# debbiemarkslab/EVcouplings

Hardware: AMD Instinct MI355X
Metric: plmc L-BFGS iterations/sec (PLM fit, synthetic MSA) (higher is better)
Workload: dtype f32 (forward: f16 hi/lo split couplings on the 2:4 sparse MFMA, f32 accumulation -- in the last iterations of a fit 39-bit fixed-point couplings as five int8 digit planes, exact; backward: 24-bit fixed-point residuals as three int8 digit planes on the int8 MFMA (32-bit / four there), exact int32 acc; 1 GPU; headline: synthetic MSA L=300 q=21 N=50000, theta=0.8, lambda_h=0.01, lambda_J=59.8; parallelism=single GPU

## Files before the change

evcouplings_amd/csrc/plm_host.cpp:

```cpp
#include "../../include/plm_hip.h"
#include "plm_internal.h"

#include <algorithm>
#include <chrono>
#include <cmath>
#include <cstdarg>
#include <cstdio>
#include <cstdlib>
#include <cstring>
#include <string>
#include <vector>

namespace {

thread_local std::string g_err;

int fail(int code, const char *fmt, ...) {
    char buf[512];
    va_list ap;
    va_start(ap, fmt);
    vsnprintf(buf, sizeof buf, fmt, ap);
    va_end(ap);
    g_err = buf;
    return code;
// ... 18 lines not shown
        hipError_t e__ = (expr);                                                                   \
        if (e__ != hipSuccess)                                                                     \
            return fail(e__ == hipErrorOutOfMemory ? PLM_ENOMEM : PLM_EDEVICE, "%s failed: %s (%s:%d)", \
                        #expr, hipGetErrorString(e__), __FILE__, __LINE__);                        \
    } while (0)
#define PLM_TRY(expr)                  \
    do {                               \
        int rc__ = (expr);             \
        if (rc__ != PLM_OK) return rc__; \
    } while (0)

double now_s() {
    return std::chrono::duration<double>(std::chrono::steady_clock::now().time_since_epoch()).count();
}

int check_device(int device) {
    int n = 0;
    if (hipGetDeviceCount(&n) != hipSuccess || n <= 0)
        return fail(PLM_EDEVICE, "no HIP device visible (libplm_hip has no CPU path)");
    if (device < 0 || device >= n) return fail(PLM_EINVAL, "device %d out of range (%d visible)", device, n);
    hipDeviceProp_t prop;
    HIP_TRY(hipGetDeviceProperties(&prop, device));
    if (strncmp(prop.gcnArchName, "gfx950", 6) != 0)
        return fail(PLM_EDEVICE, "device %d is %s; this library is built for gfx950 only", device, prop.gcnArchName);
    HIP_TRY(hipSetDevice(device));
    return PLM_OK;
}

}
int plm_check_device(int device) { return check_device(device); }
namespace {

int cluster_threshold(double theta_id, int L, int conv) {
    if (conv & PLM_CONV_THRESHOLD_F32) {
        const float t = (float)(1.0 - theta_id);
        const float need = (1.0f - t) * (float)L;
        return (int)std::ceil(need);
    }
    return (int)std::ceil(theta_id * (double)L - 1e-9);
}

}
PlmOptions plm_options_from_env() {
    PlmOptions o;
    if (const char *e = getenv("PLM_BWD_PLANES")) o.bwd_planes = atoi(e) == 4 ? 4 : 3;
    if (const char *e = getenv("PLM_KSPLIT")) o.ksplit = std::max(1, atoi(e));
    if (const char *e = getenv("PLM_JEXP_BIAS")) o.jexp_bias = atoi(e);
    if (const char *e = getenv("PLM_BWD_KERNEL")) o.bwd_kernel = atoi(e) ? 1 : 0;
    if (const char *e = getenv("PLM_FWD_KERNEL")) o.fwd_kernel = atoi(e) ? 1 : 0;
    if (const char *e = getenv("PLM_FWD_ACCURATE")) o.fwd_mode = atoi(e) ? 1 : 0;
    if (const char *e = getenv("PLM_VP_FLOOR")) o.vp_floor = atof(e);
    if (const char *e = getenv("PLM_VP_REL")) o.vp_rel = atof(e);
    if (const char *e = getenv("PLM_VP_HESS_POS")) o.vp_hess_pos = atoi(e);
    if (const char *e = getenv("PLM_ACC_FACTOR")) o.acc_factor = atof(e);
    o.debug = getenv("PLM_DEBUG") != nullptr;
    o.debug_vp = getenv("PLM_DEBUG_VP") != nullptr;
    return o;
}
namespace {

int pick_ksplit(const PlmDims &d, const PlmOptions &opt, int nplanes, int *out) {
    const int ks_min = std::max(1, (d.nst128 + 1022) / 1023);
    const int ks_max = std::max(ks_min, std::max(1, std::min(16, d.nst128 / 8)));
    if ((int64_t)((d.nst128 + ks_min - 1) / ks_min) * PLM_BWD_KSTEP * 128 * 128 >= ((int64_t)1 << 31))
        return fail(PLM_EUNSUPPORTED, "%d sequences: no admissible K split of the backward GEMM", d.N);
    const double beta = (2.0 * nplanes * (double)d.nmf * d.nnfl * 1024.0 / 12e12) / ((double)d.nst128 * 1.3e-6);
    int best = ks_min;
    double best_cost = 1e300;
    for (int ks = ks_min; ks <= ks_max; ks++) {
        const int groups_per_xcd = (d.ncol_tiles * nplanes * ks + 7) / 8;
        const double cost = (double)((groups_per_xcd * d.nrow_tiles + 31) / 32) / ks + beta * ks;
        if (cost < best_cost * 0.98) { best_cost = cost; best = ks; }
    }
    if (opt.ksplit) best = std::max(ks_min, std::min(ks_max, opt.ksplit));
    *out = best;
    return PLM_OK;
}

int make_dims(const plm_problem_t &p, const PlmOptions &opt, PlmDims *out) {
    PlmDims d;
    memset(&d, 0, sizeof d);
    if (p.n_seqs <= 0 || p.n_sites <= 1) return fail(PLM_EINVAL, "need n_seqs > 0 and n_sites > 1");
    if (!plm_q_supported(p.n_states))
        return fail(PLM_EUNSUPPORTED, "alphabet size %d outside 2..32", p.n_states);
    const int nshards = p.n_shards > 0 ? p.n_shards : 1;
    if (p.shard < 0 || p.shard >= nshards) return fail(PLM_EINVAL, "shard %d outside 0..%d", p.shard, nshards - 1);
    d.N = p.n_seqs;
    d.L = p.n_sites;
    d.Qc = p.n_states;
    d.Q = plm_q_template(p.n_states);
    d.Np = (d.N + PLM_SEQ_TILE - 1) / PLM_SEQ_TILE * PLM_SEQ_TILE;
    d.nb16 = (d.L + 15) / 16;
    d.Lp16 = d.nb16 * 16;
    d.nu = (d.L + 31) / 32;
    d.Lp32 = d.nu * 32;
    d.nksteps = d.nu * PLM_FWD_TILES(d.Q);
    d.nssteps = d.Np / 32;
    d.nst128 = d.Np / PLM_BWD_KSTEP;
    d.nplanes = (p.epsilon > 0 && p.epsilon < 1e-4) ? 4 : 3;
    if (opt.bwd_planes) d.nplanes = opt.bwd_planes;
    d.jexp_bias = opt.jexp_bias;
    const float qmax = d.nplanes == 4 ? PLM_R_QMAX4 : PLM_R_QMAX3;
    d.rscale = qmax;
    d.gscale = 1.0f / (qmax * (float)PLM_BWD_ONEHOT_VALUE);
    d.nstiles = d.Np / PLM_SEQ_TILE;
    plm_pick_tile(d.Q, &d.FM, &d.FN);
// ... 275 lines not shown
                                 plm_reg_parts(d), c->scal, c->st));
    c->n_evals++;
    return PLM_OK;
}

bool vp_enabled(const plm_ctx *c) {
    return !(c->prob.flags & PLM_FLAG_JOINT_LBFGS) && (c->d.nshards == 1 || c->d.sharded) && c->prob.lambda_h > 0;
}
int vp_alloc(plm_ctx *c) {
    if (c->hj) return PLM_OK;
    const size_t nsites = (size_t)std::max(std::max(1, (c->d.b16_hi - c->d.b16_lo) * 16),
                                           std::min(c->d.L, c->d.own_hi * 16) - c->d.h_site0);
    PLM_TRY(dalloc((char **)&c->hj, plm_hj_bytes(c->d)));
    PLM_TRY(dalloc((char **)&c->hpart, plm_hpart_bytes(c->d)));
    PLM_TRY(dalloc((char **)&c->gpart, plm_gpart_bytes(c->d)));
    PLM_TRY(dalloc((char **)&c->dpart, plm_gpart_bytes(c->d)));
    PLM_TRY(dalloc(&c->hg2, nsites));
    PLM_TRY(dalloc(&c->hinv, nsites * c->d.Q * c->d.Q));
    PLM_TRY(dalloc(&c->h64, 2 * plm_h64_stride(c->d)));
    PLM_TRY(dalloc(&c->hcnt, plm_h64_stride(c->d)));
    c->hcnt_valid = false;
    PLM_TRY(dalloc((char **)&c->vp_flag, sizeof(PlmVpState)));
    HIP_TRY(hipMemsetAsync(c->vp_flag, 0, sizeof(PlmVpState), c->st));
    for (auto &e : c->vp_ev) HIP_TRY(hipEventCreate(&e));
    for (auto &e : c->gemm_ev) HIP_TRY(hipEventCreate(&e));
    c->vp_hess_age = -1;
    return PLM_OK;
}
int vp_counts(plm_ctx *c) {
    if (!c->hcnt_valid) {
        HIP_TRY(plm_launch_site_counts(c->d, c->msa_cm, c->w, c->hcnt, c->st));
        c->hcnt_valid = true;
    }
    return PLM_OK;
}
int vp_stage1(plm_ctx *c) {
    const PlmDims &d = c->d;
    PLM_TRY(vp_counts(c));
    if (d.sharded) {
        PLM_TRY(ctx_collective(c, PLM_COLL_ALLTOALL, x_rectangles(c), c->xhalo, c->x_send.data(), c->x_recv.data()));
        HIP_TRY(plm_launch_maxabs2(c->x + d.nh_pad_l, d.n_local - d.nh_pad_l, c->xhalo,
                                   d.nx_halo * (int64_t)PLM_BLOCK_FLOATS(d), c->maxbits, c->jexp, d.jexp_bias, c->st));
        HIP_TRY(plm_launch_expand(d, c->x, c->xhalo, c->jexp, c->Bt, c->fwd_accurate ? 1 : 0, c->st));
    } else {
        HIP_TRY(plm_launch_maxabs(d, c->x, c->maxbits, c->jexp, c->st));
        HIP_TRY(plm_launch_expand(d, c->x, nullptr, c->jexp, c->Bt, c->fwd_accurate ? 1 : 0, c->st));
    }
    if (c->gemm_ev[0]) HIP_TRY(hipEventRecord(c->gemm_ev[0], c->st));
    HIP_TRY(plm_launch_forward_store(d, c->msa_rm, c->Bt, c->jexp, c->hj, c->fwd_accurate, c->st));
    HIP_TRY(plm_launch_h64_init(d, c->x, c->h64, c->st));
    return PLM_OK;
}
int vp_counts(plm_ctx *c);
int vp_step_and_residuals(plm_ctx *c, bool refresh) {
    const PlmDims &d = c->d;
    PLM_TRY(vp_counts(c));
    const int full = (refresh || c->vp_hess_age < 0) ? 1 : 0;
    HIP_TRY(plm_launch_hpass(d, c->hj, c->msa_rm, c->w, c->h64, 0, full ? 2 : 1, c->fwd_accurate, nullptr, nullptr, c->hpart,
                             c->gpart, c->dpart, nullptr, PLM_VP_ALWAYS, c->st));
    HIP_TRY(plm_launch_hsolve(d, c->hpart, c->gpart, full, c->x, c->h64, c->prob.lambda_h, 1, c->hinv, c->hg2, c->scal + 5, 0.0,
                              0.0, nullptr, 0, c->hcnt, c->dpart, c->st));
    if (full) c->vp_hess_age = 0;
    HIP_TRY(plm_launch_hpass(d, c->hj, c->msa_rm, c->w, c->h64, 1, 1, c->fwd_accurate, c->Rt, c->fx_part, c->hpart, c->gpart,
                             nullptr, nullptr, PLM_VP_ALWAYS, c->st));
    HIP_TRY(plm_launch_hsolve(d, c->hpart, c->gpart, 0, c->x, c->h64, c->prob.lambda_h, 0, c->hinv, c->hg2, c->scal + 5, 0.0,
                              0.0, nullptr, 0, c->hcnt, c->dpart, c->st));
    return PLM_OK;
}
int vp_chain(plm_ctx *c, int npos, int hess_upto, int expected_last, double tol2) {
    const PlmDims &d = c->d;
    for (int k = 0; k < npos; k++) {
        const int pos = c->vp_pos++;
        const bool hess = pos < hess_upto || pos > expected_last || c->vp_hess_age < 0;
        HIP_TRY(plm_launch_hpass(d, c->hj, c->msa_rm, c->w, c->h64, 0, hess ? 2 : 1, c->fwd_accurate, nullptr, nullptr, c->hpart,
                                 c->gpart, c->dpart, c->vp_flag, PLM_VP_PASS, c->st));
        HIP_TRY(plm_launch_hpass(d, c->hj, c->msa_rm, c->w, c->h64, 1, 1, c->fwd_accurate, c->Rt, c->fx_part, c->hpart, c->gpart,
                                 nullptr, c->vp_flag, PLM_VP_PASS_RT, c->st));
        HIP_TRY(plm_launch_hsolve(d, c->hpart, c->gpart, hess ? 2 : 0, c->x, c->h64, c->prob.lambda_h, 1, c->hinv, c->hg2,
                                  c->scal + 5, tol2, c->vp_floor2, c->vp_flag, 1, c->hcnt, c->dpart, c->st));
        if (hess && pos < 32) c->vp_hess_mask |= 1u << pos;
        if (hess && c->vp_hess_age < 0) c->vp_hess_age = 0;
    }
    return PLM_OK;
}
int vp_stage3(plm_ctx *c, bool conditional, float *gout = nullptr, int mode = 2) {
    const PlmDims &d = c->d;
    if (!gout) gout = c->g;
    if (c->gemm_ev[1]) HIP_TRY(hipEventRecord(c->gemm_ev[1], c->st));
    if (d.nblk_own > 0 || !d.sharded)
        HIP_TRY(plm_launch_backward(d, c->msa_cm, c->Rt, c->G, (conditional && !d.sharded) ? c->vp_flag : nullptr, c->st));
    if (c->gemm_ev[2]) HIP_TRY(hipEventRecord(c->gemm_ev[2], c->st));
    if (d.sharded) {
        HIP_TRY(plm_launch_pack_g(d, c->G, c->gsend, c->st));
        PLM_TRY(ctx_collective(c, PLM_COLL_ALLTOALL, c->gsend, c->ghalo, c->g_send.data(), c->g_recv.data()));
    }
    PLM_TRY(group_norms(c));
    HIP_TRY(plm_launch_assemble(d, c->G, d.ksplit, d.sharded ? c->ghalo : nullptr, c->x, gout, c->prob.lambda_h,
                                c->prob.lambda_j, c->reg_part, mode, 0.f, c->pair_n2, (float)c->prob.lambda_group, c->st));
    if (mode == 2)
        HIP_TRY(plm_launch_finish_fx(d, c->fx_part, c->n_fx_part(), nullptr, 0, c->reg_part, plm_reg_parts(d), c->scal,
                                     c->st));
    return PLM_OK;
}
int ctx_eval_vp_enqueue(plm_ctx *c, double tol2) {
    const PlmDims &d = c->d;
    PLM_TRY(vp_stage1(c));
    if (c->vp_ev_pending) c->vp_ev_pending = false;
    HIP_TRY(hipEventRecord(c->vp_ev[0], c->st));
    const int c_prev = c->vp_c_prev;
    if (c->vp_hess_age >= 0) c->vp_hess_age++;
    const bool stale = c->vp_hess_age < 0 || c->vp_hess_age >= 32;
    HIP_TRY(plm_launch_vp_reset(c->vp_flag, (c_prev == 0 && !stale) ? 1 : 0, c->scal + 5, c->st));
    c->vp_pos = 0;
    c->vp_extra = 0;
    c->vp_hess_mask = 0;
    c->vp_last_gh2 = INFINITY;
    int hess_upto = c_prev >= 2 ? c_prev : (stale ? 1 : 0);
    if (c->opt.vp_hess_pos >= 0) hess_upto = std::min(hess_upto, std::max(c->opt.vp_hess_pos, c->vp_hess_age < 0 ? 1 : 0));
    PLM_TRY(vp_chain(c, std::min(14, c_prev + 3), hess_upto, c_prev, tol2));
    HIP_TRY(plm_launch_fields_to_x(d, c->h64, c->vp_flag, c->x, c->st));
    HIP_TRY(plm_launch_hpass(d, c->hj, c->msa_rm, c->w, c->h64, 1, 0, c->fwd_accurate, c->Rt, c->fx_part, nullptr, nullptr, nullptr,
                             c->vp_flag, PLM_VP_FINAL, c->st));
    HIP_TRY(hipEventRecord(c->vp_ev[1], c->st));
    c->vp_ev_pending = true;
    PLM_TRY(vp_stage3(c, true));
    c->n_evals++;
    return PLM_OK;
// ... 1025 lines not shown
            snprintf(res->status_msg, sizeof res->status_msg, "%s", status_text(status));
    }
    return PLM_OK;
}

int plm_ctx_scores(plm_ctx_t *c, float *fn_host, float *cn_host) {
    if (!c || !fn_host || !cn_host) return fail(PLM_EINVAL, "NULL argument");
    HIP_TRY(hipSetDevice(c->device));
    const PlmDims &d = c->d;
    float *fn_dev = c->canon + d.n_canon;
    PLM_TRY(canon_full(c, c->x));
    PlmDims dc = d;
    dc.Q = d.Qc;
    if (d.gap_mode) {
        HIP_TRY(plm_launch_fn(dc, c->canon + (size_t)d.L * d.Qc, fn_dev, 1, 1, c->st));
    } else {
        HIP_TRY(plm_launch_fn(dc, c->canon + (size_t)d.L * d.Qc, fn_dev, (d.conv & PLM_CONV_FN_NO_GAP) ? 1 : 0, 0, c->st));
    }
    HIP_TRY(hipMemcpyAsync(fn_host, fn_dev, sizeof(float) * d.L * d.L, hipMemcpyDeviceToHost, c->st));
    HIP_TRY(hipStreamSynchronize(c->st));
    const int L = d.L;
    std::vector<double> col(L, 0.0);
    double tot = 0;
    for (int i = 0; i < L; i++)
        for (int j = 0; j < L; j++) {
            col[j] += fn_host[(size_t)i * L + j];
            tot += fn_host[(size_t)i * L + j];
        }
    const double mean = tot / ((double)L * (L - 1));
    for (int j = 0; j < L; j++) col[j] /= (double)(L - 1);
    for (int i = 0; i < L; i++)
        for (int j = 0; j < L; j++)
            cn_host[(size_t)i * L + j] =
                (i == j) ? 0.f : (float)((double)fn_host[(size_t)i * L + j] - col[i] * col[j] / mean);
    return PLM_OK;
}

int plm_ctx_time_field_positions(plm_ctx_t *c, int32_t reps, float *out_ms) {
    if (!c || !out_ms || reps <= 0) return fail(PLM_EINVAL, "bad argument");
    if (!c->have_weights) return fail(PLM_EINVAL, "weights not set");
    if (!vp_enabled(c) || !c->hj) return fail(PLM_EINVAL, "no stored potentials: plm_ctx_time_kernels on a variable-projection context first");
    HIP_TRY(hipSetDevice(c->device));
    const PlmDims &d = c->d;
    c->eval_valid = false;
    ctx_set_accurate(c, false);
    PLM_TRY(vp_counts(c));
    hipEvent_t ev[3] = {nullptr, nullptr, nullptr};
    for (auto &e : ev) HIP_TRY(hipEventCreate(&e));
    double acc[2] = {0, 0};
    int rc = PLM_OK;
    for (int r = 0; r < reps && rc == PLM_OK; r++) {
        float ms;
        hipError_t e = hipEventRecord(ev[0], c->st);
        if (e == hipSuccess) e = plm_launch_hpass(d, c->hj, c->msa_rm, c->w, c->h64, 0, 2, 0, nullptr, nullptr, c->hpart, c->gpart, c->dpart,
                                                  nullptr, PLM_VP_ALWAYS, c->st);
        if (e == hipSuccess) e = plm_launch_hsolve(d, c->hpart, c->gpart, 1, c->x, c->h64, c->prob.lambda_h, 1, c->hinv, c->hg2, c->scal + 5,
                                                   0.0, 0.0, nullptr, 0, c->hcnt, c->dpart, c->st);
        if (e == hipSuccess) e = hipEventRecord(ev[1], c->st);
        if (e == hipSuccess) e = plm_launch_hpass(d, c->hj, c->msa_rm, c->w, c->h64, 1, 1, 0, c->Rt, c->fx_part, c->hpart, c->gpart, nullptr,
                                                  nullptr, PLM_VP_ALWAYS, c->st);
        if (e == hipSuccess) e = plm_launch_hsolve(d, c->hpart, c->gpart, 0, c->x, c->h64, c->prob.lambda_h, 0, c->hinv, c->hg2, c->scal + 5,
                                                   0.0, 0.0, nullptr, 0, c->hcnt, c->dpart, c->st);
        if (e == hipSuccess) e = hipEventRecord(ev[2], c->st);
        if (e == hipSuccess) e = hipEventSynchronize(ev[2]);
        if (e == hipSuccess && hipEventElapsedTime(&ms, ev[0], ev[1]) == hipSuccess) acc[0] += ms;
        if (e == hipSuccess && hipEventElapsedTime(&ms, ev[1], ev[2]) == hipSuccess) acc[1] += ms;
        if (e != hipSuccess) rc = fail(PLM_EDEVICE, "field position timing: %s", hipGetErrorString(e));
    }
    for (auto &e : ev) (void)hipEventDestroy(e);
    c->vp_hess_age = 0;
    out_ms[0] = (float)(acc[0] / reps);
    out_ms[1] = (float)(acc[1] / reps);
    return rc;
}

int plm_ctx_time_kernels(plm_ctx_t *c, int32_t reps, float *out_ms) {
    if (!c || !out_ms || reps <= 0) return fail(PLM_EINVAL, "bad argument");
    if (!c->have_weights) return fail(PLM_EINVAL, "weights not set");
    if (c->d.nshards > 1 && !c->d.sharded) return fail(PLM_EUNSUPPORTED, "kernel timing runs on 1-shard or sharded-state contexts");
    HIP_TRY(hipSetDevice(c->device));
    c->eval_valid = false;
    ctx_set_accurate(c, false);
    const PlmDims &d = c->d;
    struct Events {
        hipEvent_t e[6] = {nullptr, nullptr, nullptr, nullptr, nullptr, nullptr};
        ~Events() { for (auto &x : e) if (x) (void)hipEventDestroy(x); }
    } evs;
    hipEvent_t (&ev)[6] = evs.e;
    for (auto &e : ev) HIP_TRY(hipEventCreate(&e));
    double acc[PLM_K_COUNT] = {0};
    const bool vp = vp_enabled(c);
    if (vp) PLM_TRY(vp_alloc(c));
    for (int r = 0; r < reps; r++) {
        float ms;
        HIP_TRY(hipEventRecord(ev[0], c->st));
        if (d.sharded) {
            HIP_TRY(plm_launch_maxabs2(c->x + d.nh_pad_l, d.n_local - d.nh_pad_l, c->xhalo,
                                       d.nx_halo * (int64_t)PLM_BLOCK_FLOATS(d), c->maxbits, c->jexp, d.jexp_bias, c->st));
            HIP_TRY(plm_launch_expand(d, c->x, c->xhalo, c->jexp, c->Bt, c->fwd_accurate ? 1 : 0, c->st));
        } else {
            HIP_TRY(plm_launch_maxabs(d, c->x, c->maxbits, c->jexp, c->st));
            HIP_TRY(plm_launch_expand(d, c->x, nullptr, c->jexp, c->Bt, c->fwd_accurate ? 1 : 0, c->st));
        }
        HIP_TRY(hipEventRecord(ev[1], c->st));
        if (vp) {
            HIP_TRY(plm_launch_forward_store(d, c->msa_rm, c->Bt, c->jexp, c->hj, 0, c->st));
            HIP_TRY(hipEventRecord(ev[2], c->st));
// ... 465 lines not shown
```

evcouplings_amd/csrc/plm_internal.h:

```cpp
#pragma once
#include <stdint.h>
#include <stddef.h>
#include <hip/hip_runtime.h>

#define PLM_MAX_SHARDS 16
#define PLM_PAD_STATE 127
#define PLM_SEQ_TILE 256
#define PLM_R_EXP 14
#define PLM_BWD_MAXPLANES 4
#define PLM_R_QMAX3 8355000.0f
#define PLM_R_QMAX4 2138000000.0f
#define PLM_BWD_KSTEP 128
#define PLM_BWDW_COLS 9
#define PLM_BWD_ONEHOT_VALUE (-128)

#define PLM_FWD_NG(Q) (((Q) + 2) / 4)
#define PLM_FWD_SPU(Q) (4 * PLM_FWD_NG(Q))
#define PLM_FWD_TILES(Q) (5 * PLM_FWD_NG(Q))

struct PlmDims {
    int N, L, Q;
    int Qc;
    int Np;
    int nb16;
    int Lp16;
    int nu;
    int Lp32;
    int nksteps;
    int nssteps;
    int nst128;
    int nplanes;
    float rscale;
    float gscale;
    int nstiles;
    int FM, FN;
    int nmf;
    int nshards, shard;
    int blk_per_shard;
    int shard_base, shard_rem;
    int b16_lo, b16_hi;
    int nnfl;
    int ksplit;
    int nrow_tiles, ncol_tiles;
    int fwd_w;
    int bwd_w;
    int64_t nbp;
    int64_t nh_pad;
    int64_t n_native;
    int64_t n_canon;
    int gap_mode;
    int jexp_bias;
    int conv;
    double theta;
    int sharded;
    int own_lo, own_hi;
    int nblk_own;
    int h_site0;
    int64_t bp_base;
    int64_t np_own;
    int64_t nh_pad_l;
    int64_t n_local;
    int64_t nx_halo;
    int64_t ng_halo;
    int ntri;
    int own_base[PLM_MAX_SHARDS], oth_base[PLM_MAX_SHARDS];
};

struct PlmOptions {
    int bwd_planes = 0;
    int ksplit = 0;
    int fwd_kernel = -1;
    int bwd_kernel = -1;
    int jexp_bias = 0;
    int fwd_mode = -1;
    double acc_factor = 8.0;
    double vp_rel = 1e-4;
    int vp_hess_pos = -1;
    double vp_floor = 2e-7;
    bool debug = false;
    bool debug_vp = false;
};
PlmOptions plm_options_from_env();

static inline __host__ __device__ int plm_shard_lo(const PlmDims &d, int r) {
    const int small = d.nshards - d.shard_rem;
    return r * d.shard_base + (r > small ? r - small : 0);
}
static inline __host__ __device__ int plm_shard_cnt(const PlmDims &d, int r) {
    return d.shard_base + (r >= d.nshards - d.shard_rem ? 1 : 0);
}
static inline __host__ __device__ int plm_shard_of(const PlmDims &d, int b) {
    const int small = d.nshards - d.shard_rem, nsmall = small * d.shard_base;
    if (b < nsmall) return d.shard_base > 0 ? b / d.shard_base : 0;
    return small + (b - nsmall) / (d.shard_base + 1);
}
static inline __host__ __device__ int64_t plm_bp_index(int I, int J, int nb16) {
    return (int64_t)I * nb16 - (int64_t)I * (I - 1) / 2 + (J - I);
}
static inline __host__ __device__ int plm_pair_owner(const PlmDims &d, int I, int sI, int sJ) {
    return ((I - plm_shard_lo(d, sI)) & 1) ? sJ : sI;
}
static inline __host__ __device__ int64_t plm_half_blocks(const PlmDims &d, int p) {
    return d.shard < p ? (int64_t)((d.nblk_own + 1) / 2) * plm_shard_cnt(d, p) : (int64_t)(plm_shard_cnt(d, p) / 2) * d.nblk_own;
}
static inline __host__ __device__ int64_t plm_pair_local(const PlmDims &d, int I, int J, int *halo) {
    if (halo) *halo = -1;
    if (!d.sharded) return plm_bp_index(I, J, d.nb16);
    const int sI = plm_shard_of(d, I), sJ = plm_shard_of(d, J);
    if (sI == d.shard && sJ == d.shard) {
        const int r = I - d.own_lo;
        return (int64_t)r * d.nblk_own - (int64_t)r * (r - 1) / 2 + (J - I);
    }
    if (sI != d.shard && sJ != d.shard) return -1;
    const int p = sI == d.shard ? sJ : sI;
    const int idx = ((I - plm_shard_lo(d, sI)) >> 1) * plm_shard_cnt(d, sJ) + (J - plm_shard_lo(d, sJ));
    if (plm_pair_owner(d, I, sI, sJ) == d.shard) return (int64_t)d.ntri + d.own_base[p] + idx;
    if (halo) *halo = d.oth_base[p] + idx;
    return -1;
}
static inline __host__ __device__ void plm_half_pair(const PlmDims &d, int p, bool mine, int64_t k, int *I, int *J) {
    const int np = plm_shard_cnt(d, p);
    if (d.shard < p) {
        *I = d.own_lo + 2 * (int)(k / np) + (mine ? 0 : 1);
        *J = plm_shard_lo(d, p) + (int)(k % np);
    } else {
        *I = plm_shard_lo(d, p) + 2 * (int)(k / d.nblk_own) + (mine ? 1 : 0);
        *J = d.own_lo + (int)(k % d.nblk_own);
    }
}
static inline __host__ __device__ void plm_pair_of_local(const PlmDims &d, int64_t k, int *I, int *J) {
// ... 139 lines not shown
```

evcouplings_amd/csrc/plm_kernels.hip:

```cpp
#include "../../include/plm_hip.h"
#include "plm_internal.h"
#include <math.h>
#include <stdlib.h>
#include <string.h>
#include <mutex>
#include <utility>

typedef _Float16 half8 __attribute__((ext_vector_type(8)));
typedef _Float16 half4 __attribute__((ext_vector_type(4)));
typedef _Float16 half16 __attribute__((ext_vector_type(16)));
typedef float f32x4 __attribute__((ext_vector_type(4)));
typedef int i32x4 __attribute__((ext_vector_type(4)));
typedef unsigned int u32;

#ifndef PLM_DMA_STAGGER_FWD
#define PLM_DMA_STAGGER_FWD 4
#endif
#ifndef PLM_DMA_STAGGER_BWD
#define PLM_DMA_STAGGER_BWD 0
#endif
typedef unsigned long long u64;
#ifndef PLM_ASYNC_A
#define PLM_ASYNC_A 1
#endif
// ... 1124 lines not shown
__host__ __device__ constexpr int plm_qc_min(int Q) { return Q == 4 ? 2 : Q == 5 ? 5 : Q == 20 ? 6 : Q == 21 ? 21 : 22; }
#ifndef PLM_HESS_SAMPLE
#define PLM_HESS_SAMPLE 32
#endif
#ifndef PLM_NEWTON_CAP
#define PLM_NEWTON_CAP 3.0
#endif
__device__ __forceinline__ float sum_over_g(float v) {
    unsigned u = __float_as_uint(v);
    auto a = __builtin_amdgcn_permlane32_swap(u, u, false, false);
    v = __uint_as_float(a[0]) + __uint_as_float(a[1]);
    u = __float_as_uint(v);
    auto b = __builtin_amdgcn_permlane16_swap(u, u, false, false);
    return __uint_as_float(b[0]) + __uint_as_float(b[1]);
}
__device__ __forceinline__ float log_unbiased(float z) {
    const float l2 = __builtin_amdgcn_logf(z);
    return __builtin_fmaf(l2, -1.904654323148236e-9f, l2 * 0.693147182464599609375f);
}
__device__ __forceinline__ float sel_eq(int x, int a, float if_ne, float if_eq) {
    float out;
    asm("v_cmp_eq_u32 vcc, %1, %2\n\tv_cndmask_b32 %0, %3, %4, vcc" : "=v"(out) : "s"(a), "v"(x), "v"(if_ne), "v"(if_eq) : "vcc");
    return out;
}
__device__ __forceinline__ void sel_eq2(int x, int a, float ne0, float eq0, float ne1, float eq1, float &o0, float &o1) {
    asm("v_cmp_eq_u32 vcc, %2, %3\n\tv_cndmask_b32 %0, %4, %5, vcc\n\tv_cndmask_b32 %1, %6, %7, vcc"
        : "=&v"(o0), "=&v"(o1) : "s"(a), "v"(x), "v"(ne0), "v"(eq0), "v"(ne1), "v"(eq1) : "vcc");
}
__global__ void k_sum_partials(const double *__restrict__ p, int n, double *out);
struct HpassArgs {
    const float4 *hj;
    const int8_t *msa_rm;
    const float *w;
    const double *h;
    int hstride;
    char *Rt;
    double *fx_part;
    float *hpart;
    double *gpart;
    float rscale;
    double *dpart;
    const int *state;
    int cond;
    int sel;
};
__device__ __forceinline__ bool vp_runs(const int *state, int cond) {
    if (!state || cond == PLM_VP_ALWAYS) return true;
    const PlmVpState *S = (const PlmVpState *)state;
    if (cond == PLM_VP_FINAL) return S->final_skip == 0;
    if (S->done) return false;
    return cond == PLM_VP_PASS_RT ? S->want_rt != 0 : S->want_rt == 0;
}
#define PLM_HESS_PARTS(Q) (((Q) == 20 || (Q) == 21) ? 3 : 1)
template <int Q> __host__ __device__ constexpr int hess_entry0(int a) { return a * Q - a * (a - 1) / 2; }
template <int Q> __host__ __device__ constexpr int hess_row_begin(int part) {
    if (part <= 0) return 0;
    if (part >= PLM_HESS_PARTS(Q)) return Q;
    int a = 0;
    while (a < Q && hess_entry0<Q>(a) * PLM_HESS_PARTS(Q) < part * (Q * (Q + 1) / 2)) a++;
    return a;
}
template <int Q> __host__ __device__ constexpr int hess_part_entries() {
    int m = 0;
    for (int p = 0; p < PLM_HESS_PARTS(Q); p++) {
        const int n = hess_entry0<Q>(hess_row_begin<Q>(p + 1)) - hess_entry0<Q>(hess_row_begin<Q>(p));
        m = n > m ? n : m;
    }
    return m;
}
template <int Q, bool WRITE_RT, int STATS, bool XACT>
__global__ __launch_bounds__(512) void k_hpass(PlmDims d, HpassArgs A) {
    extern __shared__ __attribute__((aligned(16))) char smem[];
    constexpr int NH = (STATS == 2) ? Q * (Q + 1) / 2 : 0;
    constexpr int NSP = (STATS == 2) ? PLM_HESS_PARTS(Q) : 1;
    constexpr int NHP = (STATS == 2) ? hess_part_entries<Q>() : 0;
    if (!vp_runs(A.state, A.cond)) return;
    if (A.state) A.h += (size_t)((const PlmVpState *)A.state)->cur * A.hstride;
    const int tid = threadIdx.x, lane = tid & 63;
    const int wave = __builtin_amdgcn_readfirstlane(tid >> 6);
    const int ns1 = (d.nstiles + PLM_HESS_SAMPLE - 1) / PLM_HESS_SAMPLE;
    const int sel = A.sel;
    const int part = (int)blockIdx.x % NSP, bid = (int)blockIdx.x / NSP;
    int row_lo = 0, row_hi = Q;
    if constexpr (NSP > 1) {
        row_lo = part == 0 ? 0 : (part == 1 ? hess_row_begin<Q>(1) : hess_row_begin<Q>(2));
        row_hi = part == 0 ? hess_row_begin<Q>(1) : (part == 1 ? hess_row_begin<Q>(2) : Q);
    }
    const int ent_lo = row_lo * Q - row_lo * (row_lo - 1) / 2, ent_hi = row_hi * Q - row_hi * (row_hi - 1) / 2;
    const int nst = sel == 0 ? d.nstiles : (sel == 1 ? ns1 : d.nstiles - ns1);
    const int kt = bid % nst, b16l = bid / nst;
    if (A.state && A.cond == PLM_VP_PASS && b16l < PLM_VP_MAXBLK && ((const PlmVpState *)A.state)->quiet[b16l]) return;
    const int stile = sel == 0 ? kt : (sel == 1 ? kt * PLM_HESS_SAMPLE : kt + kt / (PLM_HESS_SAMPLE - 1) + 1);
    constexpr int HW = Q > 21 ? 2 : 8;
    constexpr bool sampled = STATS == 2, DIAG = STATS == 3 || (STATS == 2 && Q > 21);
    const int blk = b16l * d.nstiles + stile;
    const int b16 = d.b16_lo + b16l;
    const int r = lane & 15, g = lane >> 4;
    const int s_wave = stile * PLM_SEQ_TILE + wave * 32;
    const int gap = d.gap_mode;
    const int i = b16 * 16 + r;
    const bool site_ok = i < d.L;
    float hv[XACT ? 1 : Q], hl[XACT ? 1 : Q];
    double hd[XACT ? Q : 1];
    auto load_fields = [&](bool opaque) {
        u32 hoff = (u32)(site_ok ? i - d.h_site0 : 0) * Q;
        if (opaque) asm volatile("" : "+v"(hoff));
#pragma unroll
        for (int a = 0; a < Q; a++) {
            const double h64 = site_ok ? A.h[hoff + a] : 0.0;
            if constexpr (XACT) {
                hd[a] = h64;
            } else {
                hv[a] = (float)h64;
                hl[a] = (float)(h64 - (double)hv[a]);
            }
        }
    };
    constexpr bool LDSF = !WRITE_RT && !XACT && (STATS != 2 || Q > 21);
    constexpr size_t STAT_BYTES = (size_t)16 * (8 * Q * sizeof(double) * (DIAG ? 2 : 1) + HW * NHP * sizeof(float));
    float2 *lf = (float2 *)(smem + STAT_BYTES);
    constexpr bool FAST = !WRITE_RT && !XACT && (STATS == 1 || STATS == 3);
    if constexpr (LDSF) {
        for (int k = tid; k < 16 * Q; k += 512) {
            const int ii = b16 * 16 + k / Q;
            const double h64 = ii < d.L ? A.h[(size_t)(ii - d.h_site0) * Q + k % Q] : 0.0;
            const float hi = (float)h64;
            lf[k] = make_float2(hi, (float)(h64 - (double)hi));
        }
        __syncthreads();
    } else if constexpr (!WRITE_RT) load_fields(false);
    float fxl = 0.f;
    double *lg = (double *)smem + ((size_t)wave * 16 + r) * Q;
    double *ld = lg + (size_t)8 * 16 * Q;
    float *lh0 = (float *)((double *)smem + (size_t)8 * 16 * Q * (DIAG ? 2 : 1));
    float *ls = lh0 + ((size_t)wave * 16 + r) * NHP;
    if (STATS) {
        for (int k = lane; k < 16 * Q; k += 64) ((double *)smem)[(size_t)wave * 16 * Q + k] = 0.0;
        if constexpr (sampled)
            if (wave < HW)
                for (int k = lane; k < 16 * NHP; k += 64) lh0[(size_t)wave * 16 * NHP + k] = 0.f;
        if constexpr (DIAG)
            for (int k = lane; k < 16 * Q; k += 64) ((double *)smem)[(size_t)(8 + wave) * 16 * Q + k] = 0.0;
    }
    const char *hj_u = (const char *)(A.hj + ((size_t)blk * 8 + wave) * 2 * Q * 64);
    const u32 lane16 = (u32)lane * 16;
    int m_end = 2;
    asm volatile("" : "+s"(m_end));
#pragma nounroll
    for (int m = 0; m < m_end; m++) {
        if constexpr (WRITE_RT) load_fields(true);
        f32x4 acc[Q];
#pragma unroll
        for (int a = 0; a < Q; a++) {
            const float4 v = *(const float4 *)(hj_u + (size_t)(m * Q + a) * 1024 + lane16);
            acc[a] = (f32x4){v.x, v.y, v.z, v.w};
        }
        float wk[4];
        float izk[4];
        int xk[4];
#pragma unroll
        for (int reg = 0; reg < 4; reg++) {
            const int s = s_wave + 16 * m + 4 * g + reg;
            const int xi = A.msa_rm[(size_t)s * d.Lp32 + i];
            const bool skip = gap && xi == 0;
            const float ws = (skip || !site_ok) ? 0.f : A.w[s];
            float mx = -INFINITY, Z = 0.f, hx = 0.f, zo = 0.f;
            if constexpr (!XACT) {
                u32 foff = (u32)r * Q;
                if constexpr (LDSF) asm volatile("" : "+v"(foff));
#pragma unroll
                for (int a = 0; a < Q; a++) {
                    float fh, fl;
                    if constexpr (LDSF) {
                        const float2 f = lf[foff + a];
                        fh = f.x;
                        fl = f.y;
                    } else {
                        fh = hv[a];
                        fl = hl[a];
                    }
                    const float H = ((gap && a == 0) || (a >= plm_qc_min(Q) && a >= d.Qc)) ? -INFINITY : (acc[a][reg] + fl) + fh;
                    acc[a][reg] = H;
                    mx = fmaxf(mx, H);
                }
                if constexpr (FAST) {
                    const float mxl = -mx * 1.44269502f;
#pragma unroll
                    for (int a = 0; a < Q; a++) {
                        const float ev = __builtin_amdgcn_exp2f(__builtin_fmaf(acc[a][reg], 1.44269502f, mxl));
                        const float evo = sel_eq(xi, a, ev, 0.f);
                        acc[a][reg] = evo;
                        Z += ev;
                        zo += evo;
                    }
                } else {
#pragma unroll
                    for (int a = 0; a < Q; a++) {
                        const float H = acc[a][reg] - mx;
                        const float ev = __expf(H);
                        float evo;
                        sel_eq2(xi, a, hx, H, ev, 0.f, hx, evo);
                        acc[a][reg] = ev;
                        Z += ev;
                        zo += evo;
                    }
                }
            } else {
// ... 88 lines not shown
#endif
#ifndef PLM_EXP_NOLDS
                        if (g == 0) __builtin_amdgcn_ds_faddf(LDS_FPTR(&ls[idx]), v, 0, 0, false);
#else
                        fxl += v;
#endif
                        ++idx;
                    }
                }
#endif
            }
        }
        if constexpr (WRITE_RT) {
            __builtin_amdgcn_sched_barrier(0);
            const int s64 = stile * 4 + (wave >> 1);
            const int Gq = 2 * (wave & 1) + m;
            char *rt_u = A.Rt + rt_slot(d, 0, s64, b16l * Q, 0);
            const size_t rt_plane = (size_t)d.nst128 * d.nnfl * 2048;
            const u32 slot16 = (u32)(Gq * 16 + r) * 16;
#pragma unroll
            for (int reg = 0; reg < 4; reg++) {
                wk[reg] *= A.rscale;
                asm volatile("" : "+v"(xk[reg]));
            }
            const bool four = d.nplanes == 4;
            auto planes_of_state = [&](int a, u32 (&pl)[PLM_BWD_MAXPLANES]) {
                u32 x[4];
#pragma unroll
                for (int reg = 0; reg < 4; reg++)
                    x[reg] = digits_of(wk[reg] * acc[a][reg], four);
                planes_of4(x[0], x[1], x[2], x[3], pl);
            };
#pragma unroll
            for (int q4 = 0; q4 + 4 <= Q; q4 += 4) {
                u32 pl[4][PLM_BWD_MAXPLANES];
#pragma unroll
                for (int k = 0; k < 4; k++) planes_of_state(q4 + k, pl[k]);
                const u32 off = (u32)(q4 + g) * 2048 + slot16;
#pragma unroll
                for (int p = 0; p < PLM_BWD_MAXPLANES; p++) {
                    if (p >= d.nplanes) break;
                    auto s02 = __builtin_amdgcn_permlane32_swap(pl[0][p], pl[2][p], false, false);
                    auto s13 = __builtin_amdgcn_permlane32_swap(pl[1][p], pl[3][p], false, false);
                    auto t0 = __builtin_amdgcn_permlane16_swap(s02[0], s13[0], false, false);
                    auto t1 = __builtin_amdgcn_permlane16_swap(s02[1], s13[1], false, false);
                    *(uint4 *)(rt_u + p * rt_plane + off) = make_uint4(t0[0], t0[1], t1[0], t1[1]);
                }
                __builtin_amdgcn_sched_barrier(0);
            }
#pragma unroll
            for (int a = Q - Q % 4; a < Q; a++) {
                u32 pl[PLM_BWD_MAXPLANES];
                planes_of_state(a, pl);
#pragma unroll
                for (int p = 0; p < PLM_BWD_MAXPLANES; p++)
                    if (p < d.nplanes) *(u32 *)(rt_u + p * rt_plane + (u32)a * 2048 + slot16 + 4 * g) = pl[p];
            }
        }
    }
    __syncthreads();
    if constexpr (STATS != 0) {
        if (NSP == 1 || part == 0) {
            double *gout = A.gpart + (size_t)blk * 16 * Q;
            for (int k = tid; k < 16 * Q; k += 512) {
                double v = 0;
#pragma unroll
                for (int wv = 0; wv < 8; wv++) v += ((const double *)smem)[(size_t)wv * 16 * Q + k];
                gout[k] = v;
            }
        }
        if constexpr (DIAG) {
            double *dout = A.dpart + (size_t)blk * 16 * Q;
            for (int k = tid; k < 16 * Q; k += 512) {
                double v = 0;
#pragma unroll
                for (int wv = 0; wv < 8; wv++) v += ((const double *)smem)[(size_t)(8 + wv) * 16 * Q + k];
                dout[k] = v;
            }
        }
        if constexpr (sampled) {
            float *out = A.hpart + (size_t)blk * 16 * NH;
            const int ne = ent_hi - ent_lo;
            for (int k = tid; k < 16 * ne; k += 512) {
                const int site = k / ne, e = k - site * ne;
                float v = 0.f;
#pragma unroll
                for (int wv = 0; wv < HW; wv++) v += lh0[((size_t)wv * 16 + site) * NHP + e];
                out[site * NH + ent_lo + e] = v;
            }
        }
    }
    if constexpr (WRITE_RT) {
        __syncthreads();
        const double tot = block_reduce_sum((double)fxl, (double *)smem);
        if (tid == 0) A.fx_part[blk] = tot;
    }
}
hipError_t plm_launch_hpass(const PlmDims &d, const float *hj, const int8_t *msa_rm, const float *w,
                            const double *h64, int write_rt, int stats, int exact, void *Rt, double *fx_part, float *hpart,
                            double *gpart, double *dpart, const int *state, int cond, hipStream_t st) {
    if (d.b16_hi <= d.b16_lo) return hipSuccess;
    const int nb = d.b16_hi - d.b16_lo, ns1 = (d.nstiles + PLM_HESS_SAMPLE - 1) / PLM_HESS_SAMPLE;
    const dim3 block(512);
    HpassArgs A{(const float4 *)hj, msa_rm, w, h64, (int)plm_h64_stride(d), (char *)Rt, fx_part,
                hpart, gpart, d.rscale, dpart, state, cond, 0};
#define HP_LAUNCH(QQ, WW, SS)                                                                          \
    {                                                                                                  \
        const dim3 grid((A.sel == 0 ? d.nstiles : (A.sel == 1 ? ns1 * ((SS) == 2 ? PLM_HESS_PARTS(QQ) : 1) : d.nstiles - ns1)) * nb); \
        const size_t lds = (size_t)16 * (8 * (QQ) * sizeof(double) * (((SS) == 3 || ((SS) == 2 && (QQ) > 21)) ? 2 : 1) + \
                                         ((SS) == 2 ? ((QQ) > 21 ? 2 : 8) * hess_part_entries<QQ>() : 0) * sizeof(float)) + \
                           (size_t)16 * (QQ) * sizeof(float2);           \
        {                                                                                              \
            hipError_t e = exact ? plm_allow_lds<k_hpass<QQ, WW, SS, true>>(lds) : plm_allow_lds<k_hpass<QQ, WW, SS, false>>(lds); \
            if (e != hipSuccess) return e;                                                             \
        }                                                                                              \
        if (exact) hipLaunchKernelGGL((k_hpass<QQ, WW, SS, true>), grid, block, lds, st, d, A);        \
        else hipLaunchKernelGGL((k_hpass<QQ, WW, SS, false>), grid, block, lds, st, d, A);             \
    }
#define HP_CASE(QQ)                                                                                    \
    case QQ:                                                                                           \
        if (write_rt && stats == 2) return hipErrorInvalidValue;    \
        else if (write_rt && stats == 0) HP_LAUNCH(QQ, true, 0)                                        \
        else if (write_rt) HP_LAUNCH(QQ, true, 1)                                                      \
        else if (stats == 2) {                                                                         \
            if (!dpart) return hipErrorInvalidValue;                                                   \
                         \
            A.sel = 1;                                                                                 \
            HP_LAUNCH(QQ, false, 2)                                                                    \
            A.sel = 2;                                                                                 \
            if (d.nstiles > ns1) HP_LAUNCH(QQ, false, 3)                                               \
        } else HP_LAUNCH(QQ, false, 1)                                                                 \
        break;
    switch (d.Q) {
        HP_CASE(32)
        HP_CASE(21)
        HP_CASE(20)
        HP_CASE(5)
        HP_CASE(4)
    default:
        return hipErrorInvalidValue;
    }
#undef HP_CASE
#undef HP_LAUNCH
    return hipGetLastError();
}
size_t plm_hpart_bytes(const PlmDims &d) {
    return (size_t)d.nstiles * (d.b16_hi - d.b16_lo) * 16 * (d.Q * (d.Q + 1) / 2) * sizeof(float);
}
size_t plm_h64_stride(const PlmDims &d) {
    const size_t nsites = (size_t)std::max(std::max(1, (d.b16_hi - d.b16_lo) * 16), std::min(d.L, d.own_hi * 16) - d.h_site0);
    return nsites * d.Q;
}
size_t plm_gpart_bytes(const PlmDims &d) { return (size_t)d.nstiles * (d.b16_hi - d.b16_lo) * 16 * d.Q * sizeof(double); }

template <int Q>
__global__ __launch_bounds__(256) void k_site_counts(PlmDims d, const int8_t *__restrict__ msa_cm, const float *__restrict__ w,
                                                    double *__restrict__ cnt) {
    __shared__ double red[4];
    const int il = blockIdx.x, i = d.h_site0 + il;
    double acc[Q];
#pragma unroll
    for (int a = 0; a < Q; a++) acc[a] = 0.0;
    if (i < d.L)
        for (int s = threadIdx.x; s < d.N; s += 256) {
            const int x = msa_cm[(size_t)i * d.Np + s];
            const double ws = (d.gap_mode && x == 0) ? 0.0 : (double)w[s];
#pragma unroll
            for (int a = 0; a < Q; a++) acc[a] += (x == a) ? ws : 0.0;
        }
#pragma unroll
    for (int a = 0; a < Q; a++) {
        const double t = block_reduce_sum(acc[a], red);
        if (threadIdx.x == 0) cnt[(size_t)il * Q + a] = t;
        __syncthreads();
    }
}
hipError_t plm_launch_site_counts(const PlmDims &d, const int8_t *msa_cm, const float *w, double *cnt, hipStream_t st) {
    const int nsites = (d.b16_hi - d.b16_lo) * 16;
    if (nsites <= 0) return hipSuccess;
// ... 1573 lines not shown
```

Before: 112.9 iterations/s.

## Merge sampled-Hessian and remaining-stats hpass launches into one kernel

Splits the hpass kernel into a device body and adds a combined kernel that runs the sampled Hessian tiles (stats 2) and the remaining tiles (stats 3) in one grid, branching on the workgroup index. This removes a launch and the tail gap between the two launches when the LDS footprint allows it. The change also turns on LDS-staged fields for the residual-writing pass and adds opaque-register hints on address offsets to shape code generation. The cost is that the merged launch reserves the larger of the two LDS sizes for every workgroup, which may lower occupancy for the stats-3 blocks.

Result: no change. 113.5 iterations/s (median of 3 runs) (+0.5%).

```diff
diff --git a/evcouplings_amd/csrc/plm_host.cpp b/evcouplings_amd/csrc/plm_host.cpp
--- a/evcouplings_amd/csrc/plm_host.cpp
+++ b/evcouplings_amd/csrc/plm_host.cpp
@@ -94,6 +94,7 @@
     if (const char *e = getenv("PLM_VP_FLOOR")) o.vp_floor = atof(e);
     if (const char *e = getenv("PLM_VP_REL")) o.vp_rel = atof(e);
     if (const char *e = getenv("PLM_VP_HESS_POS")) o.vp_hess_pos = atoi(e);
+    if (const char *e = getenv("PLM_VP_HESS_LAUNCHES")) o.vp_hess_launches = atoi(e) == 2 ? 2 : 1;
     if (const char *e = getenv("PLM_ACC_FACTOR")) o.acc_factor = atof(e);
     o.debug = getenv("PLM_DEBUG") != nullptr;
     o.debug_vp = getenv("PLM_DEBUG_VP") != nullptr;
@@ -475,11 +476,12 @@
     return PLM_OK;
 }
 int vp_counts(plm_ctx *c);
+static int hess_stats(const plm_ctx *c) { return c->opt.vp_hess_launches == 2 ? 2 : 4; }
 int vp_step_and_residuals(plm_ctx *c, bool refresh) {
     const PlmDims &d = c->d;
     PLM_TRY(vp_counts(c));
     const int full = (refresh || c->vp_hess_age < 0) ? 1 : 0;
-    HIP_TRY(plm_launch_hpass(d, c->hj, c->msa_rm, c->w, c->h64, 0, full ? 2 : 1, c->fwd_accurate, nullptr, nullptr, c->hpart,
+    HIP_TRY(plm_launch_hpass(d, c->hj, c->msa_rm, c->w, c->h64, 0, full ? hess_stats(c) : 1, c->fwd_accurate, nullptr, nullptr, c->hpart,
                              c->gpart, c->dpart, nullptr, PLM_VP_ALWAYS, c->st));
     HIP_TRY(plm_launch_hsolve(d, c->hpart, c->gpart, full, c->x, c->h64, c->prob.lambda_h, 1, c->hinv, c->hg2, c->scal + 5, 0.0,
                               0.0, nullptr, 0, c->hcnt, c->dpart, c->st));
@@ -495,7 +497,7 @@
     for (int k = 0; k < npos; k++) {
         const int pos = c->vp_pos++;
         const bool hess = pos < hess_upto || pos > expected_last || c->vp_hess_age < 0;
-        HIP_TRY(plm_launch_hpass(d, c->hj, c->msa_rm, c->w, c->h64, 0, hess ? 2 : 1, c->fwd_accurate, nullptr, nullptr, c->hpart,
+        HIP_TRY(plm_launch_hpass(d, c->hj, c->msa_rm, c->w, c->h64, 0, hess ? hess_stats(c) : 1, c->fwd_accurate, nullptr, nullptr, c->hpart,
                                  c->gpart, c->dpart, c->vp_flag, PLM_VP_PASS, c->st));
         HIP_TRY(plm_launch_hpass(d, c->hj, c->msa_rm, c->w, c->h64, 1, 1, c->fwd_accurate, c->Rt, c->fx_part, c->hpart, c->gpart,
                                  nullptr, c->vp_flag, PLM_VP_PASS_RT, c->st));
@@ -1627,7 +1629,7 @@
     for (int r = 0; r < reps && rc == PLM_OK; r++) {
         float ms;
         hipError_t e = hipEventRecord(ev[0], c->st);
-        if (e == hipSuccess) e = plm_launch_hpass(d, c->hj, c->msa_rm, c->w, c->h64, 0, 2, 0, nullptr, nullptr, c->hpart, c->gpart, c->dpart,
+        if (e == hipSuccess) e = plm_launch_hpass(d, c->hj, c->msa_rm, c->w, c->h64, 0, hess_stats(c), 0, nullptr, nullptr, c->hpart, c->gpart, c->dpart,
                                                   nullptr, PLM_VP_ALWAYS, c->st);
         if (e == hipSuccess) e = plm_launch_hsolve(d, c->hpart, c->gpart, 1, c->x, c->h64, c->prob.lambda_h, 1, c->hinv, c->hg2, c->scal + 5,
                                                    0.0, 0.0, nullptr, 0, c->hcnt, c->dpart, c->st);
diff --git a/evcouplings_amd/csrc/plm_internal.h b/evcouplings_amd/csrc/plm_internal.h
--- a/evcouplings_amd/csrc/plm_internal.h
+++ b/evcouplings_amd/csrc/plm_internal.h
@@ -76,6 +76,7 @@
     double acc_factor = 8.0;
     double vp_rel = 1e-4;
     int vp_hess_pos = -1;
+    int vp_hess_launches = 1;
     double vp_floor = 2e-7;
     bool debug = false;
     bool debug_vp = false;
diff --git a/evcouplings_amd/csrc/plm_kernels.hip b/evcouplings_amd/csrc/plm_kernels.hip
--- a/evcouplings_amd/csrc/plm_kernels.hip
+++ b/evcouplings_amd/csrc/plm_kernels.hip
@@ -1200,6 +1200,9 @@
     return cond == PLM_VP_PASS_RT ? S->want_rt != 0 : S->want_rt == 0;
 }
 #define PLM_HESS_PARTS(Q) (((Q) == 20 || (Q) == 21) ? 3 : 1)
+#ifndef PLM_RT_LDSF
+#define PLM_RT_LDSF 1
+#endif
 template <int Q> __host__ __device__ constexpr int hess_entry0(int a) { return a * Q - a * (a - 1) / 2; }
 template <int Q> __host__ __device__ constexpr int hess_row_begin(int part) {
     if (part <= 0) return 0;
@@ -1217,7 +1220,7 @@
     return m;
 }
 template <int Q, bool WRITE_RT, int STATS, bool XACT>
-__global__ __launch_bounds__(512) void k_hpass(PlmDims d, HpassArgs A) {
+__device__ __forceinline__ void hpass_body(const PlmDims &d, HpassArgs &A, const int wg) {
     extern __shared__ __attribute__((aligned(16))) char smem[];
     constexpr int NH = (STATS == 2) ? Q * (Q + 1) / 2 : 0;
     constexpr int NSP = (STATS == 2) ? PLM_HESS_PARTS(Q) : 1;
@@ -1228,7 +1231,7 @@
     const int wave = __builtin_amdgcn_readfirstlane(tid >> 6);
     const int ns1 = (d.nstiles + PLM_HESS_SAMPLE - 1) / PLM_HESS_SAMPLE;
     const int sel = A.sel;
-    const int part = (int)blockIdx.x % NSP, bid = (int)blockIdx.x / NSP;
+    const int part = wg % NSP, bid = wg / NSP;
     int row_lo = 0, row_hi = Q;
     if constexpr (NSP > 1) {
         row_lo = part == 0 ? 0 : (part == 1 ? hess_row_begin<Q>(1) : hess_row_begin<Q>(2));
@@ -1264,7 +1267,7 @@
             }
         }
     };
-    constexpr bool LDSF = !WRITE_RT && !XACT && (STATS != 2 || Q > 21);
+    constexpr bool LDSF = !XACT && (!WRITE_RT || PLM_RT_LDSF);
     constexpr size_t STAT_BYTES = (size_t)16 * (8 * Q * sizeof(double) * (DIAG ? 2 : 1) + HW * NHP * sizeof(float));
     float2 *lf = (float2 *)(smem + STAT_BYTES);
     constexpr bool FAST = !WRITE_RT && !XACT && (STATS == 1 || STATS == 3);
@@ -1296,11 +1299,14 @@
     asm volatile("" : "+s"(m_end));
 #pragma nounroll
     for (int m = 0; m < m_end; m++) {
-        if constexpr (WRITE_RT) load_fields(true);
+        if constexpr (WRITE_RT && !LDSF) load_fields(true);
         f32x4 acc[Q];
+        const char *hj_m = hj_u + (size_t)m * Q * 1024;
+        u32 hoff = lane16;
+        if constexpr (WRITE_RT) asm volatile("" : "+v"(hoff));
 #pragma unroll
         for (int a = 0; a < Q; a++) {
-            const float4 v = *(const float4 *)(hj_u + (size_t)(m * Q + a) * 1024 + lane16);
+            const float4 v = *(const float4 *)(hj_m + (size_t)a * 1024 + hoff);
             acc[a] = (f32x4){v.x, v.y, v.z, v.w};
         }
         float wk[4];
@@ -1495,9 +1501,11 @@
             for (int a = Q - Q % 4; a < Q; a++) {
                 u32 pl[PLM_BWD_MAXPLANES];
                 planes_of_state(a, pl);
+                u32 toff = (u32)a * 2048 + slot16 + 4 * g;
+                asm volatile("" : "+v"(toff));
 #pragma unroll
                 for (int p = 0; p < PLM_BWD_MAXPLANES; p++)
-                    if (p < d.nplanes) *(u32 *)(rt_u + p * rt_plane + (u32)a * 2048 + slot16 + 4 * g) = pl[p];
+                    if (p < d.nplanes) *(u32 *)(rt_u + p * rt_plane + toff) = pl[p];
             }
         }
     }
@@ -1537,6 +1545,40 @@
         __syncthreads();
         const double tot = block_reduce_sum((double)fxl, (double *)smem);
         if (tid == 0) A.fx_part[blk] = tot;
+    }
+}
+template <int Q, bool WRITE_RT, int STATS, bool XACT>
+__global__ __launch_bounds__(512) void k_hpass(PlmDims d, HpassArgs A) {
+    hpass_body<Q, WRITE_RT, STATS, XACT>(d, A, (int)blockIdx.x);
+}
+template <int Q>
+__global__ __launch_bounds__(512) void k_hpass_hess(PlmDims d, HpassArgs A, int n_sampled) {
+    const int wg = (int)blockIdx.x;
+    if (wg < n_sampled) {
+        A.sel = 1;
+        hpass_body<Q, false, 2, false>(d, A, wg);
+    } else {
+        A.sel = 2;
+        hpass_body<Q, false, 3, false>(d, A, wg - n_sampled);
+    }
+}
+template <int Q> constexpr size_t hpass_lds_bytes(int stats) {
+    return (size_t)16 * (8 * Q * sizeof(double) * ((stats == 3 || (stats == 2 && Q > 21)) ? 2 : 1) +
+                         (stats == 2 ? (Q > 21 ? 2 : 8) * hess_part_entries<Q>() : 0) * sizeof(float)) +
+           (size_t)16 * Q * sizeof(float2);
+}
+template <int Q> constexpr bool hpass_hess_merges() { return 2 * hpass_lds_bytes<Q>(2) <= 160 * 1024; }
+template <int Q>
+static hipError_t hpass_launch_hess(const PlmDims &d, const HpassArgs &A, int nb, int ns1, hipStream_t st) {
+    if constexpr (hpass_hess_merges<Q>()) {
+        const int n_sampled = ns1 * PLM_HESS_PARTS(Q) * nb;
+        const size_t lds = std::max(hpass_lds_bytes<Q>(2), hpass_lds_bytes<Q>(3));
+        const hipError_t e = plm_allow_lds<k_hpass_hess<Q>>(lds);
+        if (e != hipSuccess) return e;
+        hipLaunchKernelGGL((k_hpass_hess<Q>), dim3(n_sampled + (d.nstiles - ns1) * nb), dim3(512), lds, st, d, A, n_sampled);
+        return hipSuccess;
+    } else {
+        return hipErrorInvalidValue;
     }
 }
 hipError_t plm_launch_hpass(const PlmDims &d, const float *hj, const int8_t *msa_rm, const float *w,
@@ -1547,12 +1589,12 @@
     const dim3 block(512);
     HpassArgs A{(const float4 *)hj, msa_rm, w, h64, (int)plm_h64_stride(d), (char *)Rt, fx_part,
                 hpart, gpart, d.rscale, dpart, state, cond, 0};
+    const bool one_launch = stats == 4 && !exact && d.nstiles > ns1;
+    if (stats == 4) stats = 2;
 #define HP_LAUNCH(QQ, WW, SS)                                                                          \
     {                                                                                                  \
         const dim3 grid((A.sel == 0 ? d.nstiles : (A.sel == 1 ? ns1 * ((SS) == 2 ? PLM_HESS_PARTS(QQ) : 1) : d.nstiles - ns1)) * nb); \
-        const size_t lds = (size_t)16 * (8 * (QQ) * sizeof(double) * (((SS) == 3 || ((SS) == 2 && (QQ) > 21)) ? 2 : 1) + \
-                                         ((SS) == 2 ? ((QQ) > 21 ? 2 : 8) * hess_part_entries<QQ>() : 0) * sizeof(float)) + \
-                           (size_t)16 * (QQ) * sizeof(float2);           \
+        const size_t lds = hpass_lds_bytes<QQ>(SS);                                                    \
         {                                                                                              \
             hipError_t e = exact ? plm_allow_lds<k_hpass<QQ, WW, SS, true>>(lds) : plm_allow_lds<k_hpass<QQ, WW, SS, false>>(lds); \
             if (e != hipSuccess) return e;                                                             \
@@ -1567,7 +1609,12 @@
         else if (write_rt) HP_LAUNCH(QQ, true, 1)                                                      \
         else if (stats == 2) {                                                                         \
             if (!dpart) return hipErrorInvalidValue;                                                   \
-                         \
+            if (one_launch && hpass_hess_merges<QQ>()) {                                               \
+                const hipError_t e = hpass_launch_hess<QQ>(d, A, nb, ns1, st);                         \
+                if (e != hipSuccess) return e;                                                         \
+                break;                                                                                 \
+            }                                                                                          \
+             \
             A.sel = 1;                                                                                 \
             HP_LAUNCH(QQ, false, 2)                                                                    \
             A.sel = 2;                                                                                 \
```
